# SauersML/genomic_pca

Measured on AMD Instinct MI355X. Metric: SNPs x samples / sec through rSVD at k=20; max|dPC| vs ref, higher is better.
Workload: dtype i8 (exact: int8 dosages x 4 signed 7-bit fixed-point digit planes of the skinny operand, i32 accumulate, f64 recombination; accuracy >= f32)

## Files before the change

### genomic_pca_amd/_lib.py

```python
from __future__ import annotations

import ctypes as C
import os
import subprocess

_PKG = os.path.dirname(os.path.abspath(__file__))
LIB_PATH = os.path.join(_PKG, "libgpca.so")
CSRC = os.path.join(_PKG, "csrc")

GPCA_OK = 0
GPCA_ERR_BAD_ARG = -1
GPCA_ERR_OOM = -2
GPCA_ERR_HIP = -3
GPCA_ERR_RCCL = -4
GPCA_ERR_MISSING_GENOTYPE = -5
GPCA_ERR_NOT_CONVERGED = -6
GPCA_ERR_STATE = -7
GPCA_ERR_NO_DEVICE = -8
GPCA_ERR_INVALID_GENOTYPE = -9
GPCA_UNIQUE_ID_BYTES = 128
PREC_DEFAULT = 0
PREC_I8_EXACT = 1
PREC_F32_MFMA = 2
STORE_AUTO = 0
STORE_2BIT = 1
STORE_INT8 = 2
GRM_STANDARDIZED = 0
GRM_CENTRED = 1
CFG_SIMPLE_KERNELS = 1
CFG_NO_COMPACT = 2
CFG_NO_NARROW = 4
CFG_NO_SPIN_SYNC = 8


class GpcaLibraryError(RuntimeError):
    pass


class GpcaError(RuntimeError):
    def __init__(self, status: int, message: str):
        super().__init__(f"[gpca status {status}] {message}")
        self.status = status
        self.message = message


class gpca_config(C.Structure):
    _fields_ = [("device", C.c_int32), ("precision", C.c_int32), ("storage", C.c_int32), ("digit_planes", C.c_int32),
# ... 137 lines not shown
```

### genomic_pca_amd/csrc/gemm_i8.hip

```cpp
#include "gemm_i8_common.h"

namespace gpca {

template <int NSU>
struct GqnG { i32x4 g[4 * NSU]; float r, b; };
template <int NSU>
__device__ __forceinline__ void gqn_load(GqnG<NSU>& b, const int8_t* __restrict__ G, int64_t ldg, int64_t unit, int c, int h,
                                         const float* __restrict__ rv, const float* __restrict__ bv) {
    const __amdgpu_buffer_rsrc_t rg = make_rsrc8(G + unit * 32 * ldg);
    const uint32_t vo = (uint32_t)(c * ldg + 16 * h);
#pragma unroll
    for (int j = 0; j < 4 * NSU; ++j) b.g[j] = __builtin_amdgcn_raw_buffer_load_b128(rg, vo, 32u * j, 2);
    b.r = rv[unit * 32 + c]; b.b = bv[unit * 32 + c];
}
template <int NSU, int PF>
__global__ __launch_bounds__(256, 1) void k_gq_n(const int8_t* __restrict__ G, int64_t ldg, int64_t units,
                                                  const int8_t* __restrict__ Qd, const double* __restrict__ qscale,
                                                  const float* __restrict__ rv, const float* __restrict__ bv,
                                                  const float* __restrict__ sv, float* __restrict__ Tout,
                                                  float* __restrict__ cunit, double* __restrict__ apart, int scale_out, int64_t ldt) {
    const int lane = threadIdx.x & 63;
    const int wv = __builtin_amdgcn_readfirstlane(threadIdx.x >> 6);
    const int c = lane & 31, h = lane >> 5;
    const int64_t wave = (int64_t)blockIdx.x * 4 + wv, waves = (int64_t)gridDim.x * 4;
// ... 591 lines not shown
    if (h == 0) apart[((int64_t)blockIdx.x * 4 + wv) * 32 + c] = (double)am;
}

int launch_gq_d(hipStream_t st, const int8_t* G, int64_t ldg, const GqPlan& plan, int64_t Npad, const int8_t* Qd,
                const double* qscale, const float* r, const float* b, const float* s, float* Tout, float* cpart, double* apart,
                int scale_out, int64_t ldt, const KernelOpts& ko) {
    if (!dma_shape_ok(Npad, 256, plan.units * 32, 32) || ldg < Npad) return (int)hipErrorInvalidValue;
    const dim3 grid((unsigned)(plan.waves / 4)), blk(256);
    const int64_t nstage = Npad / 128;
    int phase = ko.gq_phase;
    if (phase < 0) phase = (nstage >= 16 && nstage <= 400) ? (int)((nstage / 8) << 16) : 0;
    hipLaunchKernelGGL((k_gq_d<1>), grid, blk, sizeof(GqdSmem), st, G, ldg, plan.units, nstage, Qd, qscale, r, b, s, Tout, cpart, apart, scale_out, ldt, ko.gq_chain, phase);
    return 0;
}

template <bool PACKED>
struct GttXG { unsigned g[16]; };

#ifndef GPCA_GTTX_AUX
#define GPCA_GTTX_AUX 2
#endif
template <bool PACKED>
__device__ __forceinline__ void gttx_load_g(GttXG<PACKED>& b, __amdgpu_buffer_rsrc_t rg, uint32_t gvo, uint32_t row_off, uint32_t ldr) {
#pragma unroll
    for (int i = 0; i < 16; ++i) b.g[i] = (unsigned)__builtin_amdgcn_raw_buffer_load_b32(rg, gvo, row_off + (uint32_t)i * ldr, PACKED ? 0 : GPCA_GTTX_AUX);
}
template <bool PACKED, int ABL = 0>
__device__ __forceinline__ void gttx_decode_step(const GttXG<PACKED>& bn, Gtt2Ops& on, unsigned (&x)[4], unsigned (&y)[4], int m, unsigned bsh) {
    const int w = m >> 2, ph = m & 3;
    if (ABL & 1) { on.bt[ph][w] = (int)bn.g[4 * w + ph]; return; }
// ... 365 lines not shown

int launch_gtt_d(hipStream_t st, const int8_t* G, int64_t ldg, int64_t Mpad, int64_t Npad, const int8_t* Td, double* Ypart,
                 const Gtt8Plan& plan, const KernelOpts& ko) {
    if (plan.tasks_per_wg < 1 || plan.S * 128 != Mpad || !dma_shape_ok(Npad, 256, Mpad, kGQRowsPerWave) || ldg < Npad) return (int)hipErrorInvalidValue;
    const dim3 grid((unsigned)plan.grid), blk(256);
    const int remap = ko.gtt_xcd;
    hipLaunchKernelGGL((k_gtt_d<1>), grid, blk, sizeof(GqdSmem), st, (const uint8_t*)G, ldg, Npad, Td, Ypart, plan.S, plan.C, plan.ngroups, plan.W, plan.tasks_per_wg, plan.strided, remap);
    return 0;
}

int init_device_kernels_i8() {
    int e = 0;
#define GPCA_OPT_IN(KERNEL, BYTES) \
    if (e == 0) e = (int)hipFuncSetAttribute(reinterpret_cast<const void*>(KERNEL), hipFuncAttributeMaxDynamicSharedMemorySize, (int)(BYTES));
    GPCA_OPT_IN((k_gq_d<1>), sizeof(GqdSmem))
    GPCA_OPT_IN((k_gtt_p<kDigits>), sizeof(GtpSmem)) GPCA_OPT_IN((k_gtt_p<3>), sizeof(GtpSmem))
    GPCA_OPT_IN((k_gtt_d<1>), sizeof(GqdSmem))
#undef GPCA_OPT_IN
    return e;
}

}
```

### genomic_pca_amd/csrc/gpca_api.cpp

```cpp
#include "gpca_internal.h"

using namespace gpca;

RcclApi g_rccl;
thread_local std::string g_last_global_err;

static thread_local uint64_t g_tls_err_gen = 0;
static thread_local std::string g_tls_err;
static std::atomic<uint64_t> g_next_gen{1};
int fail(gpca_handle* h, int code, const std::string& msg) {
    if (h) { h->err = msg; g_tls_err_gen = h->gen; g_tls_err = msg; } else g_last_global_err = msg;
    return code;
}

void fold_timings(gpca_handle* h) {
    for (auto& r : h->recs) {
        float ms = 0.f;
        if (hipEventSynchronize(r.b) == hipSuccess && hipEventElapsedTime(&ms, r.a, r.b) == hipSuccess) {
            size_t i = 0;
            for (; i < h->agg.size(); ++i) if (r.name == h->agg[i].name) break;
            if (i == h->agg.size()) { gpca_kernel_timing t{}; snprintf(t.name, sizeof t.name, "%s", r.name.c_str()); h->agg.push_back(t); }
            h->agg[i].launches++; h->agg[i].total_ms += ms; h->agg[i].flops += r.flops; h->agg[i].bytes += r.bytes;
        }
        h->ev_pool.push_back(r.a); h->ev_pool.push_back(r.b);
// ... 41 lines not shown
    h->storage_cfg = cfg ? cfg->storage : GPCA_STORE_AUTO;
    if (h->storage_cfg != GPCA_STORE_AUTO && h->storage_cfg != GPCA_STORE_INT8 && h->storage_cfg != GPCA_STORE_2BIT) { delete h; return fail(nullptr, GPCA_ERR_BAD_ARG, "gpca_create: unknown storage mode"); }
    if (h->precision != GPCA_PREC_F32_MFMA && h->precision != GPCA_PREC_I8_EXACT) { delete h; return fail(nullptr, GPCA_ERR_BAD_ARG, "gpca_create: unknown precision mode"); }
    h->storage = h->storage_cfg == GPCA_STORE_2BIT ? GPCA_STORE_2BIT : GPCA_STORE_INT8;
    {
        const int dp = cfg ? cfg->digit_planes : 0;
        if (dp != 0 && dp != 3 && dp != 4) { delete h; return fail(nullptr, GPCA_ERR_BAD_ARG, "gpca_create: digit_planes must be 0, 3 or 4"); }
        if (dp == 3 && !(h->precision == GPCA_PREC_I8_EXACT && h->storage_cfg == GPCA_STORE_2BIT)) { delete h; return fail(nullptr, GPCA_ERR_BAD_ARG, "gpca_create: digit_planes = 3 is implemented for GPCA_PREC_I8_EXACT with GPCA_STORE_2BIT"); }
        h->nd_cfg = dp;
        h->nd = dp == 3 ? 3 : ((dp == 0 && h->precision == GPCA_PREC_I8_EXACT && h->storage == GPCA_STORE_2BIT) ? 3 : 4);
    }
    {
        const int32_t flags = cfg ? cfg->reserved[0] : 0, gqw = cfg ? cfg->reserved[1] : 0, gtw = cfg ? cfg->reserved[2] : 0;
        if ((flags & ~GPCA_CFG_ALL) != 0 || gqw < 0 || gtw < 0 || (cfg && cfg->reserved[3] != 0)) { delete h; return fail(nullptr, GPCA_ERR_BAD_ARG, "gpca_create: unknown bits in gpca_config.reserved"); }
        h->simple_kernels = (flags & GPCA_CFG_SIMPLE_KERNELS) != 0;
        h->compact_ok = (flags & GPCA_CFG_NO_COMPACT) == 0;
        h->narrow_ok = (flags & GPCA_CFG_NO_NARROW) == 0;
        h->spin_sync = (flags & GPCA_CFG_NO_SPIN_SYNC) == 0;
        if (gqw) h->gq_waves_target = std::max(4, (int)gqw);
        if (gtw) h->gtt_waves_target = std::max(4, (int)gtw);
    }
    if (hipSetDevice(dev) != hipSuccess || hipStreamCreateWithFlags(&h->st, hipStreamNonBlocking) != hipSuccess) {
        delete h; return fail(nullptr, GPCA_ERR_HIP, "gpca_create: hipSetDevice/hipStreamCreate failed");
    }
    hipDeviceProp_t prop;
    if (hipGetDeviceProperties(&prop, dev) == hipSuccess) {
        if (strncmp(prop.gcnArchName, "gfx950", 6) != 0) {
            std::string m = std::string("gpca_create: device is ") + prop.gcnArchName + ", this library only carries gfx950 code";
            (void)hipStreamDestroy(h->st); delete h; return fail(nullptr, GPCA_ERR_NO_DEVICE, m);
        }
// ... 468 lines not shown
```

### genomic_pca_amd/csrc/gpca_internal.h

```cpp
#pragma once
#include "../../include/gpca.h"
#include "kernels.h"

#include <dlfcn.h>
#include <hip/hip_runtime.h>

#include <algorithm>
#include <atomic>
#include <chrono>
#include <condition_variable>
#include <deque>
#include <thread>
#include <cmath>
#include <cstdio>
#include <cstdlib>
#include <cstring>
#include <map>
#include <mutex>
#include <string>
#include <vector>

using namespace gpca;

typedef struct ncclComm* ncclComm_t;
// ... 142 lines not shown
        hipStream_t st = nullptr;
        hipEvent_t dep = nullptr;
        int64_t *d_rows = nullptr, *d_cols = nullptr; float* d_out = nullptr; unsigned long long* d_err = nullptr;
        size_t cap_rows = 0, cap_cols = 0, cap_out = 0;
    };
    std::mutex pull_mu;
    std::condition_variable pull_cv;
    std::vector<PullLane*> lanes_free;
    int lanes_total = 0;
    std::atomic<int> pulls_in_flight{0};
    double *dYpart64 = nullptr, *d_qscale = nullptr, *d_qinv = nullptr, *d_tscale = nullptr, *d_tinv = nullptr;
    size_t cap_Qd = 0, cap_Td = 0, cap_Ypart64 = 0;
    int nd = 4;
    uint64_t gen = 0;
    int simple_kernels = 0;
    int narrow_ok = 1;
    int gq_waves_target = 1024, gtt_waves_target = 2048;

    gpca_handle* child = nullptr;
    bool child_valid = false, rsvd_on_child = false;
    bool is_child = false;
    const int64_t* d_row_ids = nullptr;
    int compact_ok = 1;

    int world = 1, rank = 0;
    int64_t snp_offset = 0;
    ncclComm_t comm = nullptr;
    gpca_allreduce_fn hook = nullptr;
    void* hook_user = nullptr;
    std::vector<double> hook_buf;
// ... 168 lines not shown
```

### genomic_pca_amd/csrc/gpca_rsvd.cpp

```cpp
#include "gpca_internal.h"

using namespace gpca;

static void tred2(int n, double* V, double* d, double* e) {
    for (int j = 0; j < n; ++j) d[j] = V[(n - 1) * n + j];
    for (int i = n - 1; i > 0; --i) {
        double scale = 0.0, h = 0.0;
        for (int k = 0; k < i; ++k) scale += std::fabs(d[k]);
        if (scale == 0.0) {
            e[i] = d[i - 1];
            for (int j = 0; j < i; ++j) { d[j] = V[(i - 1) * n + j]; V[i * n + j] = 0.0; V[j * n + i] = 0.0; }
        } else {
            for (int k = 0; k < i; ++k) { d[k] /= scale; h += d[k] * d[k]; }
            double f = d[i - 1];
            double g = std::sqrt(h);
            if (f > 0) g = -g;
            e[i] = scale * g; h -= f * g; d[i - 1] = f - g;
            for (int j = 0; j < i; ++j) e[j] = 0.0;
            for (int j = 0; j < i; ++j) {
                f = d[j]; V[j * n + i] = f; g = e[j] + V[j * n + j] * f;
                for (int k = j + 1; k <= i - 1; ++k) { g += V[k * n + j] * d[k]; e[k] += V[k * n + j] * f; }
                e[j] = g;
            }
            f = 0.0;
// ... 122 lines not shown
    return GPCA_OK;
}


static inline bool narrow_shape(const gpca_handle* h) {
    return h->narrow_ok && h->precision == GPCA_PREC_I8_EXACT && h->storage == GPCA_STORE_INT8 && h->N <= kNarrowSamples;
}
static inline bool k2_batched(const gpca_handle* h) {
    return !narrow_shape(h) && !h->simple_kernels;
}
static inline Gtt8Plan k2_plan(const gpca_handle* h, int64_t rows_pad) {
    return narrow_shape(h) ? gtt8_plan_narrow(rows_pad, h->N, std::min(h->gtt_waves_target, 1024)) :
           k2_batched(h) ? gtt8_plan_batched(rows_pad, h->ldg, h->gtt_waves_target) : gtt8_plan(rows_pad, h->ldg, h->gtt_waves_target);
}

static inline GqPlan k1_plan(const gpca_handle* h, int64_t rows_pad) { return gq_plan(rows_pad, h->gq_waves_target); }

static int k2_panel(gpca_handle* h, const PanelView& pv, const int8_t* Td_half, const Gtt8Plan& plan) {
    const int8_t* Td = Td_half + (size_t)(pv.row0 >> 5) * kPlaneBytesPerBlock;
    const bool packed = h->storage == GPCA_STORE_2BIT;
    if (narrow_shape(h)) launch_gtt_n(h->st, pv.g8, h->ld8, pv.rows_pad, h->ldg, Td, h->dYpart64, plan);
    else if (h->simple_kernels) {
        if (packed) launch_gtt_2bit(h->st, pv.g2, h->ld2, pv.rows_pad, h->ldg, Td, h->dYpart64, plan, h->nd);
        else launch_gtt_i8(h->st, pv.g8, h->ld8, pv.rows_pad, h->ldg, Td, h->dYpart64, plan, h->ko);
    } else if (packed) {
        const int e = launch_gtt_p(h->st, pv.g2, h->ld2, pv.rows_pad, h->ldg, Td, h->dYpart64, plan, h->nd, h->ko);
        if (e != 0) return fail(h, GPCA_ERR_HIP, "k_gtt_p launch failed (hip error " + std::to_string(e) + ")");
    } else {
        const int e = launch_gtt_d(h->st, pv.g8, h->ld8, pv.rows_pad, h->ldg, Td, h->dYpart64, plan, h->ko);
        if (e != 0) return fail(h, GPCA_ERR_HIP, "k_gtt_d launch failed (hip error " + std::to_string(e) + ")");
// ... 56 lines not shown

static int stage_AQ(gpca_handle* h, int scale_out) {
    const double elems = (double)h->M * (double)h->N;
    if (h->precision == GPCA_PREC_I8_EXACT) {
        const int L = h->L, halves = L / 32;
        const bool packed = h->storage == GPCA_STORE_2BIT, streamed = h->sm.on;
        const size_t qhalf = (size_t)h->ldg * 32 * kDigits;
        const size_t chalf = (size_t)h->Mpad;
        const size_t ahalf = (size_t)h->gqplan.waves * 32;
        if (streamed && scale_out) HIPCHK(hipMemsetAsync(h->d_amax_run, 0, kMaxSketch * 8, h->st));
        {
            const double by = packed ? elems / 4 : elems;
            ScopedTimer sweep(h, "gemm_GQ", 2.0 * elems * h->l, by * halves, nullptr, streamed);
            CHK(for_each_panel(h, [&](const PanelView& pv) -> int {
                const GqPlan plan = streamed ? k1_plan(h, pv.rows_pad) : h->gqplan;
                for (int hf = 0; hf < halves; ++hf) {
                    const int8_t* Qd = h->dQd + hf * qhalf;
                    const double* qsc = h->d_qscale + 32 * hf;
                    const float* s32 = h->d_s32 + 32 * hf;
                    const float* rr = h->d_r + pv.row0; const float* bb = h->d_b + pv.row0;
                    float* Th = h->dT + (size_t)pv.row0 * L + 32 * hf;
                    float* cp = h->d_cpart + hf * chalf + (size_t)pv.row0;
                    double* ap = h->d_apart + hf * ahalf;
                    ScopedTimer t(h, "gemm_GQ", 2.0 * elems * h->l / halves, by, nullptr, !streamed);
                    if (packed) launch_gq_2bit(h->st, pv.g2, h->ld2, plan, h->ldg, Qd, qsc, rr, bb, s32, Th, cp, ap, scale_out, h->nd, L);
                    else if (narrow_shape(h)) {
                        const int e = launch_gq_n(h->st, pv.g8, h->ld8, plan, h->N, Qd, qsc, rr, bb, s32, Th, cp, ap, scale_out, L);
                        if (e != 0) return fail(h, GPCA_ERR_HIP, "k_gq_n launch failed (hip error " + std::to_string(e) + ")");
                    }
                    else if (!h->simple_kernels) {
                        const int e = launch_gq_d(h->st, pv.g8, h->ld8, plan, h->ldg, Qd, qsc, rr, bb, s32, Th, cp, ap, scale_out, L, h->ko);
                        if (e != 0) return fail(h, GPCA_ERR_HIP, "k_gq_d launch failed (hip error " + std::to_string(e) + ")");
                    }
                    else launch_gq_i8(h->st, pv.g8, h->ld8, plan, h->N, Qd, qsc, rr, bb, s32, Th, cp, scale_out, L, h->ko);
                    HIPCHK(hipGetLastError());
                    if (streamed && scale_out && (packed || !h->simple_kernels || narrow_shape(h))) {
                        launch_absmax_fold(h->st, ap, plan.waves, h->d_amax_run + 32 * hf);
                        HIPCHK(hipGetLastError());
                    }
                }
                return GPCA_OK;
            }));
        }
        h->apart_valid = scale_out != 0 && (packed || !h->simple_kernels || narrow_shape(h));
        h->c_fold_pending = scale_out != 0 && !streamed && h->apart_valid;
        if (scale_out)
            for (int hf = 0; hf < halves; ++hf) {
                if (h->c_fold_pending)
                    launch_post_k1(h->st, h->d_cpart + hf * chalf, h->Mpad / 32, h->d_scratch64 + (size_t)hf * kPostK1Scratch, h->d_apart + hf * ahalf, h->gqplan.waves,
                                   h->d_tscale + 32 * hf, h->d_tinv + 32 * hf, h->nd);
                else launch_sum_partials_f32(h->st, h->d_cpart + hf * chalf, h->Mpad / 32, 32, h->d_c + 32 * hf, h->d_scratch64);
                HIPCHK(hipGetLastError());
            }
        for (int hf = 0; hf < kMaxSketch / 32; ++hf) h->apart_src[hf] = streamed ? h->d_amax_run + 32 * hf : h->d_apart + hf * ahalf;
// ... 12 lines not shown
}

static int stage_power_fused(gpca_handle* h) {
    const double elems = (double)h->M * (double)h->N;
    const int L = h->L, halves = L / 32;
    const bool packed = h->storage == GPCA_STORE_2BIT;
    const size_t qhalf = (size_t)h->ldg * 32 * kDigits, chalf = (size_t)h->Mpad, ahalf = (size_t)h->gqplan.waves * 32;
    const size_t td_half = (size_t)h->Mpad * 32 * kDigits, yint_half = (size_t)h->N * 32;
    {
        const double by = packed ? elems / 4 : elems;
        ScopedTimer sweep(h, "gemm_fused", 4.0 * elems * h->l, by * halves);
        CHK(for_each_panel(h, [&](const PanelView& pv) -> int {
            const GqPlan plan1 = k1_plan(h, pv.rows_pad);
            const Gtt8Plan plan2 = k2_plan(h, pv.rows_pad);
            const float* rr = h->d_r + pv.row0; const float* bb = h->d_b + pv.row0;
            for (int hf = 0; hf < halves; ++hf) {
                const int8_t* Qd = h->dQd + hf * qhalf;
                float* Th = h->dT + (size_t)pv.row0 * L + 32 * hf;
                float* cp = h->d_cpart + hf * chalf + (size_t)pv.row0;
                double* ap = h->d_apart + hf * ahalf;
                if (packed) launch_gq_2bit(h->st, pv.g2, h->ld2, plan1, h->ldg, Qd, h->d_qscale + 32 * hf, rr, bb, h->d_s32 + 32 * hf, Th, cp, ap, 1, h->nd, L);
                else if (narrow_shape(h)) {
                    const int e = launch_gq_n(h->st, pv.g8, h->ld8, plan1, h->N, Qd, h->d_qscale + 32 * hf, rr, bb, h->d_s32 + 32 * hf, Th, cp, ap, 1, L);
                    if (e != 0) return fail(h, GPCA_ERR_HIP, "k_gq_n launch failed (hip error " + std::to_string(e) + ")");
                }
                else {
                    const int e = launch_gq_d(h->st, pv.g8, h->ld8, plan1, h->ldg, Qd, h->d_qscale + 32 * hf, rr, bb, h->d_s32 + 32 * hf, Th, cp, ap, 1, L, h->ko);
                    if (e != 0) return fail(h, GPCA_ERR_HIP, "k_gq_d launch failed (hip error " + std::to_string(e) + ")");
                }
                HIPCHK(hipGetLastError());
                launch_quantize_f32_premax(h->st, Th, pv.rows_pad, pv.rows_pad, ap, plan1.waves, h->d_tscale + 32 * hf, h->d_tinv + 32 * hf,
                                           h->dTd + hf * td_half + (size_t)(pv.row0 >> 5) * kPlaneBytesPerBlock, 0, h->nd, L);
                HIPCHK(hipGetLastError());
            }
            for (int hf = 0; hf < halves; ++hf) {
                CHK(k2_panel(h, pv, h->dTd + hf * td_half, plan2));
                launch_accum_y_scaled(h->st, h->dYpart64, plan2.W, h->ldg, h->N, h->d_tscale + 32 * hf, h->d_yint + hf * yint_half, pv.index == 0);
                HIPCHK(hipGetLastError());
            }
            return GPCA_OK;
        }));
    }
    for (int hf = 0; hf < halves; ++hf) {
        launch_sum_partials_f32(h->st, h->d_cpart + hf * chalf, h->Mpad / 32, 32, h->d_c + 32 * hf, h->d_scratch64);
        HIPCHK(hipGetLastError());
        launch_finish_y_sum(h->st, h->d_yint + hf * yint_half, h->N, h->d_c + 32 * hf, h->dY + 32 * hf, L);
        HIPCHK(hipGetLastError());
    }
// ... 220 lines not shown
    return 2 * npad <= h->Mpad;
}
static int ensure_child(gpca_handle* h) {
    if (h->child && h->child_valid) return GPCA_OK;
    drop_child(h);
    const bool packed = h->storage == GPCA_STORE_2BIT;
    const int64_t n = h->n_pca, npad = round_up(n, kGQRowsPerWave), pitch = packed ? h->ld2 : h->ld8;
    size_t free_b = 0, total_b = 0;
    HIPCHK(hipMemGetInfo(&free_b, &total_b));
    const double need = (double)npad * (double)pitch + (double)npad * 1024.0 + (double)h->ldg * 8192.0 + 1073741824.0;
    if (need > (double)free_b) return GPCA_ERR_OOM;
    gpca_handle* c = new gpca_handle();
    c->is_child = true; c->compact_ok = 0;
    c->device = h->device; c->precision = h->precision; c->storage = h->storage; c->nd = h->nd; c->ko = h->ko;
    c->st = h->st;
    c->simple_kernels = h->simple_kernels; c->narrow_ok = h->narrow_ok; c->spin_sync = h->spin_sync;
    c->gq_waves_target = h->gq_waves_target; c->gtt_waves_target = h->gtt_waves_target;
    c->timing_on = h->timing_on;
    c->M = n; c->N = h->N; c->Mpad = npad; c->ldg = h->ldg; c->ld8 = h->ld8; c->ld2 = h->ld2; c->cap_rows_pad = npad; c->pack_flags = h->pack_flags;
    h->child = c;
    auto build = [&]() -> int {
        gpca_handle* hh = h;
        (void)hh;
        if (packed) { HIPCHK(malloc_genotypes(h, (void**)&c->dG2, (size_t)npad * (size_t)pitch)); }
        else { HIPCHK(malloc_genotypes(h, (void**)&c->dG, (size_t)npad * (size_t)pitch)); }
        char* gdst = packed ? (char*)c->dG2 : (char*)c->dG;
        if (npad > n) HIPCHK(hipMemsetAsync(gdst + (size_t)n * pitch, 0, (size_t)(npad - n) * pitch, h->st));
        launch_gather_rows(h->st, packed ? (const void*)h->dG2 : (const void*)h->dG, pitch, h->d_pca_rows, n, gdst);
        HIPCHK(hipGetLastError());
        {
            gpca_handle* h = c;
// ... 378 lines not shown
```

### genomic_pca_amd/csrc/kernels.h

```cpp
#pragma once
#include <hip/hip_runtime.h>
#include <stdint.h>
#include "eig_result.h"
#include "plan_math.h"

namespace gpca {

struct QcParams { double min_call_rate, min_maf, max_hwe_p; };

struct KernelOpts {
    int gq_phase = -1;
    int gq_chain = 1;
    int gtt_xcd = 1;
};
int init_device_kernels_i8();
int init_device_kernels_common();
int init_device_kernels_eig();

void launch_small_eigh(hipStream_t st, const double* src, int nslices, int n, int L, int k, int zmode, double denom, const int* cholflag,
                       double* Z, double* res, double* Vout);

__host__ __device__ inline int64_t blocked_t_index(int64_t row, int col, int LT) {
    const int64_t group = row >> 4;
    const int w = (int)(row & 15), lt = col >> 5, cc = col & 31;
// ... 137 lines not shown
void launch_quantize_f64_prescaled(hipStream_t st, const double* X, int64_t rows, int64_t rows_pad, const double* inv, int8_t* Xd, int layout, int nd = 4, int64_t ldx = 32);
void launch_quantize_f64_finishq(hipStream_t st, const double* X, int64_t rows, int64_t rows_pad, int8_t* Xd, int layout, int nd, int64_t ldx,
                                 const double* csum_part, const double* amax_part, int64_t P, int ldp, double* s64, float* s32, double* scale, double* inv);
void launch_quantize_f32_premax(hipStream_t st, const float* X, int64_t rows, int64_t rows_pad, const double* apart, int64_t P,
                                double* scale, double* inv, int8_t* Xd, int layout, int nd = 4, int64_t ldx = 32);
void launch_post_k1(hipStream_t st, const float* cpart, int64_t units, double* cscratch, const double* apart, int64_t P, double* scale, double* inv, int nd);
void launch_quantize_f32_cfold(hipStream_t st, const float* X, int64_t rows, int64_t rows_pad, const double* inv, int8_t* Xd, int layout, int nd,
                               int64_t ldx, const double* cscratch, int cslices, double* c);
int launch_gtt_p(hipStream_t st, const uint8_t* G2, int64_t ld2, int64_t Mpad, int64_t Npad, const int8_t* Td, double* Ypart,
                 const Gtt8Plan& plan, int nd = 4, const KernelOpts& ko = KernelOpts());
int launch_gtt_d(hipStream_t st, const int8_t* G, int64_t ldg, int64_t Mpad, int64_t Npad, const int8_t* Td, double* Ypart,
                 const Gtt8Plan& plan, const KernelOpts& ko = KernelOpts());
int launch_gq_d(hipStream_t st, const int8_t* G, int64_t ldg, const GqPlan& plan, int64_t Npad, const int8_t* Qd,
                const double* qscale, const float* r, const float* b, const float* s, float* Tout, float* cpart, double* apart,
                int scale_out, int64_t ldt = 32, const KernelOpts& ko = KernelOpts());
void launch_gtt_2bit(hipStream_t st, const uint8_t* G2, int64_t ld2, int64_t Mpad, int64_t Npad, const int8_t* Td,
                     double* Ypart, const Gtt8Plan& plan, int nd = 4);


void launch_project(hipStream_t st, const void* G, int packed, int64_t ldr, int64_t Mpad, int64_t Npad, const int8_t* Ta, const int8_t* Tb,
                    const uint32_t* rmask, double* Ypa, double* Ypb, unsigned* cnt, unsigned* bad, const PrjPlan& plan, int nd, int lazy_b);
void launch_project_correct(hipStream_t st, const double* Yint_b, int64_t N, const double* tscale_b, const unsigned* cnt, int64_t n_model,
                            double* Y, int64_t ldy);
void launch_project_colmax(hipStream_t st, const float* X, int64_t rows, int L, unsigned long long* out);
void launch_project_used(hipStream_t st, const unsigned* cnt, int64_t N, double n_model, double* used);

constexpr int kGrmDigits = 6;
constexpr int kGrmFlushRows = 4096;
constexpr int kGrmTabBytes = 4 * kGrmDigits * 32;
void launch_grm(hipStream_t st, const void* G, int packed, int64_t ldr, int64_t rows_pad, const int8_t* tab, const uint32_t* kmask,
// ... 52 lines not shown
```

### include/gpca.h

```cpp
#ifndef GPCA_H
#define GPCA_H

#include <stddef.h>
#include <stdint.h>

#if defined(__GNUC__)
#define GPCA_API __attribute__((visibility("default")))
#else
#define GPCA_API
#endif

#ifdef __cplusplus
extern "C" {
#endif

#define GPCA_VERSION 250
#define GPCA_MISSING_I8 (-127)

typedef struct gpca_handle gpca_handle;

typedef enum gpca_status {
    GPCA_OK = 0,
    GPCA_ERR_BAD_ARG = -1,
    GPCA_ERR_OOM = -2,
// ... 17 lines not shown
    GPCA_STORE_2BIT = 1,
    GPCA_STORE_INT8 = 2
} gpca_storage;

typedef struct gpca_config {
    int32_t device;
    int32_t precision;
    int32_t storage;
    int32_t digit_planes;
    int32_t reserved[4];
} gpca_config;
#define GPCA_CFG_SIMPLE_KERNELS 1
#define GPCA_CFG_NO_COMPACT 2
#define GPCA_CFG_NO_NARROW 4
#define GPCA_CFG_NO_SPIN_SYNC 8
#define GPCA_CFG_ALL 15

typedef struct gpca_qc_config {
    double min_snp_call_rate;
    double min_snp_maf;
    double max_snp_hwe_p_value;
} gpca_qc_config;

GPCA_API int gpca_version(void);
GPCA_API const char* gpca_status_string(int status);
GPCA_API int gpca_create(const gpca_config* cfg, gpca_handle** out);
GPCA_API int gpca_destroy(gpca_handle* h);
GPCA_API const char* gpca_last_error(gpca_handle* h);

GPCA_API int gpca_upload_genotypes_i8(gpca_handle* h, const int8_t* snp_major, int64_t M, int64_t N, int64_t ld);
GPCA_API int gpca_upload_bed2bit(gpca_handle* h, const uint8_t* bed_rows, int64_t M, int64_t N);
// ... 141 lines not shown
```

Before: 964.7 billion.

## Fuse both Q column halves into one int8 GEMM pass over genotypes

Adds a k_gq_d2 kernel that computes the G·Q product for two 32-column halves of the skinny operand in a single sweep over the int8 genotype matrix. Before, each half launched its own kernel that re-read G. The intent is to halve genotype memory traffic on the memory-bound first GEMM of each rSVD iteration. The new kernel has its own LDS layout, a slot-based DMA pipeline with compile-time audited vmcnt waits, and chaining across rounds. It runs by default for int8 non-narrow storage, with a config flag to fall back to per-half launches. The cost is a larger LDS footprint, more accumulator registers per wave, and a complex hand-tuned wait schedule.

Result: no change. 964.7 billion (median of 2 runs) (+0.0%).

```diff
diff --git a/genomic_pca_amd/_lib.py b/genomic_pca_amd/_lib.py
--- a/genomic_pca_amd/_lib.py
+++ b/genomic_pca_amd/_lib.py
@@ -31,6 +31,7 @@
 CFG_NO_COMPACT = 2
 CFG_NO_NARROW = 4
 CFG_NO_SPIN_SYNC = 8
+CFG_K1_PER_HALF = 16
 
 
 class GpcaLibraryError(RuntimeError):
diff --git a/genomic_pca_amd/csrc/gemm_i8.hip b/genomic_pca_amd/csrc/gemm_i8.hip
--- a/genomic_pca_amd/csrc/gemm_i8.hip
+++ b/genomic_pca_amd/csrc/gemm_i8.hip
@@ -1,4 +1,5 @@
 #include "gemm_i8_common.h"
+#include "gqd2_counts.h"
 
 namespace gpca {
 
@@ -629,6 +630,247 @@
     return 0;
 }
 
+struct Gqd2Smem {
+    i32x4 q[2][kGqd2Blocks][4][kDigits][64];
+    i32x4 g[4][kGqd2Slots][256];
+    float tile[4][32 * 32];
+    float rb[4][2][32 * kGqd2MaxR];
+    double colq[4][kGqd2Blocks][32];
+    float cols[4][kGqd2Blocks][32];
+};
+static_assert(sizeof(Gqd2Smem) <= 160 * 1024, "LDS of one CU");
+static_assert(kGqd2MaxR * kGqd2Blocks * kDigits * 16 == 256, "accumulators of a wave");
+static_assert(32 * kGqd2MaxR <= 64, "r and b of a round's rows: one 64-dword DMA each");
+
+__device__ __forceinline__ void gqd2_wait_young(int batches) {
+    switch (batches) {
+        case 1: gqd_wait_vm<gqd2_young_wait(1)>(); break;
+        case 2: gqd_wait_vm<gqd2_young_wait(2)>(); break;
+        default: gqd_wait_vm<gqd2_young_wait(3)>(); break;
+    }
+}
+static_assert(gqd2_q_young(1, 0) <= 3 && gqd2_q_young(2, 0) <= 3 && gqd2_q_young(2, 1) >= 1 && gqd2_q_young_early(1) >= 1, "cases of gqd2_wait_young");
+
+template <int NT, int R>
+__device__ __forceinline__ void gqd2_round(const int8_t* __restrict__ G, int64_t ldg, int64_t nstage,
+                                           const int8_t* __restrict__ Qd0, const int8_t* __restrict__ Qd1, Gqd2Smem* sm, int wv, int lane, int c, int h,
+                                           int64_t unit0, int nvalid, bool prologue, bool chain, GqdRound nx, uint32_t& rslot, uint32_t ph,
+                                           int64_t rows_total, const float* __restrict__ rv,
+                                           const float* __restrict__ bv, float* __restrict__ Tout, int scale_out, int64_t ldt,
+                                           float* __restrict__ cunit, int64_t c_stride, float (&amax)[kGqd2Blocks]) {
+    constexpr int S = kGqd2Slots, B = kGqd2Blocks;
+    static_assert(R >= 1 && R <= kGqd2MaxR, "tiles per wave");
+    auto phys = [&](uint32_t st_) -> uint32_t { const uint32_t p_ = st_ + ph; return p_ >= (uint32_t)nstage ? p_ - (uint32_t)nstage : p_; };
+    const int64_t row0 = unit0 * 32;
+    const i32x4 rg = gqd_rsrc(G + row0 * ldg);
+    const i32x4 rgn = gqd_rsrc(G + nx.unit0 * 32 * ldg);
+    const i32x4 rq0 = gqd_rsrc(Qd0 + wv * 1024), rq1 = gqd_rsrc(Qd1 + wv * 1024);
+    const uint32_t ld32 = (uint32_t)ldg;
+    const uint32_t gvo_e = (uint32_t)(lane >> 3) * ld32 + 16u * (uint32_t)((lane & 7) ^ (lane >> 4));
+    const uint32_t gvo_o = (uint32_t)(lane >> 3) * ld32 + 16u * (uint32_t)((lane & 7) ^ (lane >> 4) ^ 4);
+    const uint32_t qvo = (uint32_t)(lane * 16);
+    uint32_t toff[R];
+#pragma unroll
+    for (int t = 0; t < R; ++t) toff[t] = (uint32_t)(t < nvalid ? 32 * t : 0) * ld32;
+    {
+        const uint32_t lds_rb = (uint32_t)(uintptr_t)(__attribute__((address_space(3))) void*)&sm->rb[wv][0][0];
+        i32x4 rr_ = gqd_rsrc(rv + row0), rb_ = gqd_rsrc(bv + row0);
+        rr_.z = rb_.z = (int)((rows_total - row0) * 4);
+        asm volatile("s_waitcnt lgkmcnt(0)" ::: "memory");
+        gqd_dma_dword(lds_rb, qvo >> 2, rr_, 0u);
+        gqd_dma_dword(lds_rb + 4u * 32u * kGqd2MaxR, qvo >> 2, rb_, 0u);
+    }
+    constexpr uint32_t QCH = kDigits * 1024;
+    const uint32_t lds_q = (uint32_t)(uintptr_t)(__attribute__((address_space(3))) void*)&sm->q[0][0][0][0][0] + (uint32_t)wv * 1024u;
+    const uint32_t lds_g = (uint32_t)(uintptr_t)(__attribute__((address_space(3))) void*)&sm->g[0][0][0] + (uint32_t)wv * (S * 4096u);
+    const char* gl = reinterpret_cast<const char*>(&sm->g[wv][0][0]);
+    uint32_t loff[4];
+#pragma unroll
+    for (int s4 = 0; s4 < 4; ++s4) loff[s4] = (uint32_t)(c * 128 + (((2 * s4 + h) ^ ((c >> 1) & 7)) * 16));
+
+    i32x16 acc[R][B][kDigits];
+#pragma unroll
+    for (int t = 0; t < R; ++t)
+#pragma unroll
+        for (int b = 0; b < B; ++b)
+#pragma unroll
+            for (int d = 0; d < kDigits; ++d)
+#pragma unroll
+                for (int e = 0; e < 16; ++e) acc[t][b][d][e] = 0;
+
+#define GQD2_ISSUE_G(RSRC, SO, SLOT)                                                                      \
+    {                                                                                                     \
+        const uint32_t so_ = (SO);                                                                        \
+        const uint32_t la_ = lds_g + (uint32_t)(SLOT) * 4096u;                                            \
+        _Pragma("unroll") for (int i = 0; i < kGqd2FillDmas; ++i) gqd_dma<NT>(la_ + 1024u * i, (i & 1) ? gvo_o : gvo_e, RSRC, so_ + 8u * i * ld32); \
+    }
+#define GQD2_ISSUE_Q(ST, QS)                                                                              \
+    {                                                                                                     \
+        const uint32_t sq_ = phys((uint32_t)(ST)) * 4u;                                                   \
+        _Pragma("unroll") for (int j = 0; j < 4; ++j)                                                     \
+            gqd_dma(lds_q + (uint32_t)((((QS) * B + 0) * 4 + j) * kDigits) * 1024u, qvo, rq0, (sq_ + j) * QCH); \
+        _Pragma("unroll") for (int j = 0; j < 4; ++j)                                                     \
+            gqd_dma(lds_q + (uint32_t)((((QS) * B + 1) * 4 + j) * kDigits) * 1024u, qvo, rq1, (sq_ + j) * QCH); \
+    }
+    int64_t ist = 0;
+    int it = 0;
+    bool in_next = false;
+    uint32_t pst = 0; int pt = 0;
+#define GQD2_ISSUE_NEXT(SLOT)                                                                             \
+    {                                                                                                     \
+        if (!in_next) {                                                                                   \
+            GQD2_ISSUE_G(rg, toff[it] + phys((uint32_t)ist) * 128u, SLOT)                                 \
+            if (++it == R) { it = 0; if (++ist == nstage) { if (chain) in_next = true; else ist = 0; } }  \
+        } else {                                                                                          \
+            const uint32_t tn_ = (uint32_t)(pt < nx.nv ? 32 * pt : 0) * ld32;                             \
+            GQD2_ISSUE_G(rgn, tn_ + phys(pst) * 128u, SLOT)                                               \
+            if (++pt == nx.R) { pt = 0; ++pst; }                                                          \
+        }                                                                                                 \
+    }
+    if (prologue) {
+        rslot = 0;
+#pragma unroll
+        for (int sl = 0; sl < S - 2; ++sl) GQD2_ISSUE_NEXT(sl)
+        GQD2_ISSUE_Q(0, 0)
+#pragma unroll
+        for (int sl = S - 2; sl < S; ++sl) GQD2_ISSUE_NEXT(sl)
+    } else {
+        ist = S / R; it = S % R;
+    }
+    i32x4 gcur, gnxt;
+
+    for (int64_t st = 0; st < nstage; ++st) {
+        asm volatile("s_waitcnt vmcnt(%0)\n\ts_barrier" :: "n"(gqd2_stage_wait(R)) : "memory");
+        GQD2_ISSUE_Q(st + 1 < nstage ? st + 1 : 0, (int)((st + 1) & 1))
+        i32x4 q[B][4][kDigits];
+#pragma unroll
+        for (int b = 0; b < B; ++b)
+#pragma unroll
+            for (int s4 = 0; s4 < 4; ++s4)
+#pragma unroll
+                for (int d = 0; d < kDigits; ++d) q[b][s4][d] = sm->q[st & 1][b][s4][d][lane];
+        if (st == 0) {
+            gcur = *reinterpret_cast<const i32x4*>(gl + rslot * 4096u + loff[0]);
+            gnxt = *reinterpret_cast<const i32x4*>(gl + rslot * 4096u + loff[1]);
+        }
+#pragma unroll
+        for (int t = 0; t < R; ++t) {
+            const char* ub = gl + rslot * 4096u;
+            const uint32_t nslot = rslot == S - 1 ? 0u : rslot + 1u;
+#pragma unroll
+            for (int s4 = 0; s4 < 4; ++s4) {
+                i32x4 gfar;
+                if (s4 < 2) {
+                    gfar = *reinterpret_cast<const i32x4*>(ub + loff[s4 + 2]);
+                } else {
+                    if (s4 == 2) {
+                        if (st < gqd2_early_stages(R)) gqd2_wait_young(gqd2_q_young_early(R));
+                        else gqd2_wait_young(gqd2_q_young(R, t));
+                    }
+                    gfar = *reinterpret_cast<const i32x4*>(gl + nslot * 4096u + loff[s4 - 2]);
+                }
+#pragma unroll
+                for (int b = 0; b < B; ++b)
+#pragma unroll
+                    for (int d = 0; d < kDigits; ++d)
+                        acc[t][b][d] = __builtin_amdgcn_mfma_i32_32x32x32_i8(gcur, q[b][s4][d], acc[t][b][d], 0, 0, 0);
+                if (s4 == 3) {
+                    asm volatile("" :: "v"(gcur));
+                    GQD2_ISSUE_NEXT(rslot)
+                }
+                gcur = gnxt; gnxt = gfar;
+            }
+            rslot = nslot;
+        }
+    }
+    if (!chain) asm volatile("s_waitcnt vmcnt(0)\n\ts_barrier" ::: "memory");
+#undef GQD2_ISSUE_NEXT
+#undef GQD2_ISSUE_G
+#undef GQD2_ISSUE_Q
+    float* tile = sm->tile[wv];
+#pragma unroll
+    for (int t = 0; t < R; ++t)
+        if (t < nvalid) {
+#pragma unroll
+            for (int b = 0; b < B; ++b)
+                gq_tile_out<7, true>(acc[t][b], 0.f, 0.f, &sm->rb[wv][0][32 * t], &sm->rb[wv][1][32 * t], sm->colq[wv][b][c], sm->cols[wv][b][c], scale_out, tile, Tout + 32 * b, ldt, unit0 + t,
+                                     cunit + b * c_stride, amax[b], lane, nx.unit0 != unit0);
+        }
+}
+
+template <int NT>
+__global__ __launch_bounds__(256, 1) void k_gq_d2(const int8_t* __restrict__ G, int64_t ldg, int64_t units, int64_t nstage,
+                                                   const int8_t* __restrict__ Qd, int64_t qd_stride, const double* __restrict__ qscale,
+                                                   const float* __restrict__ rv, const float* __restrict__ bv,
+                                                   const float* __restrict__ sv, float* __restrict__ Tout,
+                                                   float* __restrict__ cpart, int64_t c_stride, double* __restrict__ apart, int64_t a_stride,
+                                                   int scale_out, int64_t ldt, int chain_ok, int phase_mul) {
+    extern __shared__ __attribute__((aligned(16))) char gqd_smem[];
+    Gqd2Smem* sm = reinterpret_cast<Gqd2Smem*>(gqd_smem);
+    __builtin_assume(nstage >= 2 && (nstage & 1) == 0);
+    const int wv = __builtin_amdgcn_readfirstlane(threadIdx.x >> 6);
+    const uint32_t ph = (uint32_t)(((int64_t)(blockIdx.x & 7) * (phase_mul & 0xffff) + (int64_t)(blockIdx.x >> 3) * (phase_mul >> 16)) % nstage);
+    const int64_t u0 = (units * (int64_t)blockIdx.x) / gridDim.x;
+    const int64_t u1 = (units * ((int64_t)blockIdx.x + 1)) / gridDim.x;
+    float amax[kGqd2Blocks] = {0.f, 0.f};
+    {
+        const int l0 = threadIdx.x & 63;
+        sm->colq[wv][l0 >> 5][l0 & 31] = qscale[l0];
+        sm->cols[wv][l0 >> 5][l0 & 31] = sv[l0];
+    }
+    auto round_at = [&](int64_t u) -> GqdRound {
+        const int64_t rem = u1 - u, take = rem < kGqd2RoundUnits ? rem : kGqd2RoundUnits;
+        const int base = (int)(take >> 2), extra = (int)(take & 3);
+        const int nv = base + (wv < extra ? 1 : 0);
+        GqdRound r;
+        r.nv = nv; r.R = nv ? nv : 1;
+        r.unit0 = nv ? u + wv * base + (wv < extra ? wv : extra) : u;
+        return r;
+    };
+    const bool chain_all = chain_ok && nstage > kGqd2Slots;
+    uint32_t rslot = 0;
+    int64_t u = u0;
+    while (u < u1) {
+        const int64_t un = u + (u1 - u < kGqd2RoundUnits ? u1 - u : kGqd2RoundUnits);
+        const GqdRound cur = round_at(u);
+        const bool chain = chain_all && un < u1;
+        const bool prologue = !chain_all || u == u0;
+        GqdRound nx = cur;
+        if (chain) nx = round_at(un);
+        int lane;
+        asm volatile("v_mbcnt_lo_u32_b32 %0, -1, 0\n\tv_mbcnt_hi_u32_b32 %0, -1, %0" : "=v"(lane));
+        const int c = lane & 31, h = lane >> 5;
+#define GPCA_GQD2_ROUND(RR) gqd2_round<NT, RR>(G, ldg, nstage, Qd, Qd + qd_stride, sm, wv, lane, c, h, cur.unit0, cur.nv, prologue, chain, nx, rslot, ph, units * 32, rv, bv, Tout, scale_out, ldt, cpart, c_stride, amax)
+        if (cur.R == 2) GPCA_GQD2_ROUND(2);
+        else GPCA_GQD2_ROUND(1);
+#undef GPCA_GQD2_ROUND
+        u = un;
+    }
+#pragma unroll
+    for (int b = 0; b < kGqd2Blocks; ++b) {
+        float am_lo, am_hi; halves_pair(amax[b], am_lo, am_hi);
+        const float am = fmaxf(am_lo, am_hi);
+        int l0;
+        asm volatile("v_mbcnt_lo_u32_b32 %0, -1, 0\n\tv_mbcnt_hi_u32_b32 %0, -1, %0" : "=v"(l0));
+        if (l0 < 32) apart[b * a_stride + ((int64_t)blockIdx.x * 4 + wv) * 32 + l0] = (double)am;
+    }
+}
+
+int launch_gq_d2(hipStream_t st, const int8_t* G, int64_t ldg, const GqPlan& plan, int64_t Npad, const int8_t* Qd, int64_t qd_stride,
+                 const double* qscale, const float* r, const float* b, const float* s, float* Tout, float* cpart, int64_t c_stride,
+                 double* apart, int64_t a_stride, int scale_out, int64_t ldt, const KernelOpts& ko) {
+    if (!dma_shape_ok(Npad, 256, plan.units * 32, 32) || ldg < Npad) return (int)hipErrorInvalidValue;
+    if (ldt < 32 * kGqd2Blocks || qd_stride < Npad * 32 * kDigits || qd_stride % 1024 != 0) return (int)hipErrorInvalidValue;
+    if (c_stride < plan.units * 32 || a_stride < plan.waves * 32 || plan.waves < 4 || plan.waves % 4 != 0) return (int)hipErrorInvalidValue;
+    const dim3 grid((unsigned)(plan.waves / 4)), blk(256);
+    const int64_t nstage = Npad / 128;
+    int phase = ko.gq_phase;
+    if (phase < 0) phase = (nstage >= 16 && nstage <= 400) ? (int)((nstage / 8) << 16) : 0;
+    hipLaunchKernelGGL((k_gq_d2<1>), grid, blk, sizeof(Gqd2Smem), st, G, ldg, plan.units, nstage, Qd, qd_stride, qscale, r, b, s, Tout, cpart, c_stride, apart, a_stride,
+                       scale_out, ldt, ko.gq_chain, phase);
+    return 0;
+}
+
 template <bool PACKED>
 struct GttXG { unsigned g[16]; };
 
@@ -1024,6 +1266,7 @@
 #define GPCA_OPT_IN(KERNEL, BYTES) \
     if (e == 0) e = (int)hipFuncSetAttribute(reinterpret_cast<const void*>(KERNEL), hipFuncAttributeMaxDynamicSharedMemorySize, (int)(BYTES));
     GPCA_OPT_IN((k_gq_d<1>), sizeof(GqdSmem))
+    GPCA_OPT_IN((k_gq_d2<1>), sizeof(Gqd2Smem))
     GPCA_OPT_IN((k_gtt_p<kDigits>), sizeof(GtpSmem)) GPCA_OPT_IN((k_gtt_p<3>), sizeof(GtpSmem))
     GPCA_OPT_IN((k_gtt_d<1>), sizeof(GqdSmem))
 #undef GPCA_OPT_IN
diff --git a/genomic_pca_amd/csrc/gpca_api.cpp b/genomic_pca_amd/csrc/gpca_api.cpp
--- a/genomic_pca_amd/csrc/gpca_api.cpp
+++ b/genomic_pca_amd/csrc/gpca_api.cpp
@@ -79,6 +79,7 @@
         const int32_t flags = cfg ? cfg->reserved[0] : 0, gqw = cfg ? cfg->reserved[1] : 0, gtw = cfg ? cfg->reserved[2] : 0;
         if ((flags & ~GPCA_CFG_ALL) != 0 || gqw < 0 || gtw < 0 || (cfg && cfg->reserved[3] != 0)) { delete h; return fail(nullptr, GPCA_ERR_BAD_ARG, "gpca_create: unknown bits in gpca_config.reserved"); }
         h->simple_kernels = (flags & GPCA_CFG_SIMPLE_KERNELS) != 0;
+        h->k1_per_half = (flags & GPCA_CFG_K1_PER_HALF) != 0;
         h->compact_ok = (flags & GPCA_CFG_NO_COMPACT) == 0;
         h->narrow_ok = (flags & GPCA_CFG_NO_NARROW) == 0;
         h->spin_sync = (flags & GPCA_CFG_NO_SPIN_SYNC) == 0;
diff --git a/genomic_pca_amd/csrc/gpca_internal.h b/genomic_pca_amd/csrc/gpca_internal.h
--- a/genomic_pca_amd/csrc/gpca_internal.h
+++ b/genomic_pca_amd/csrc/gpca_internal.h
@@ -180,6 +180,7 @@
     int nd = 4;
     uint64_t gen = 0;
     int simple_kernels = 0;
+    int k1_per_half = 0;
     int narrow_ok = 1;
     int gq_waves_target = 1024, gtt_waves_target = 2048;
 
diff --git a/genomic_pca_amd/csrc/gpca_rsvd.cpp b/genomic_pca_amd/csrc/gpca_rsvd.cpp
--- a/genomic_pca_amd/csrc/gpca_rsvd.cpp
+++ b/genomic_pca_amd/csrc/gpca_rsvd.cpp
@@ -160,6 +160,9 @@
            k2_batched(h) ? gtt8_plan_batched(rows_pad, h->ldg, h->gtt_waves_target) : gtt8_plan(rows_pad, h->ldg, h->gtt_waves_target);
 }
 
+static inline bool k1_one_read(const gpca_handle* h) {
+    return h->storage != GPCA_STORE_2BIT && !narrow_shape(h) && !h->simple_kernels && !h->k1_per_half;
+}
 static inline GqPlan k1_plan(const gpca_handle* h, int64_t rows_pad) { return gq_plan(rows_pad, h->gq_waves_target); }
 
 static int k2_panel(gpca_handle* h, const PanelView& pv, const int8_t* Td_half, const Gtt8Plan& plan) {
@@ -246,7 +249,8 @@
             ScopedTimer sweep(h, "gemm_GQ", 2.0 * elems * h->l, by * halves, nullptr, streamed);
             CHK(for_each_panel(h, [&](const PanelView& pv) -> int {
                 const GqPlan plan = streamed ? k1_plan(h, pv.rows_pad) : h->gqplan;
-                for (int hf = 0; hf < halves; ++hf) {
+                for (int hf = 0, nb = 1; hf < halves; hf += nb) {
+                    nb = (k1_one_read(h) && hf + 1 < halves) ? 2 : 1;
                     const int8_t* Qd = h->dQd + hf * qhalf;
                     const double* qsc = h->d_qscale + 32 * hf;
                     const float* s32 = h->d_s32 + 32 * hf;
@@ -254,8 +258,12 @@
                     float* Th = h->dT + (size_t)pv.row0 * L + 32 * hf;
                     float* cp = h->d_cpart + hf * chalf + (size_t)pv.row0;
                     double* ap = h->d_apart + hf * ahalf;
-                    ScopedTimer t(h, "gemm_GQ", 2.0 * elems * h->l / halves, by, nullptr, !streamed);
-                    if (packed) launch_gq_2bit(h->st, pv.g2, h->ld2, plan, h->ldg, Qd, qsc, rr, bb, s32, Th, cp, ap, scale_out, h->nd, L);
+                    ScopedTimer t(h, "gemm_GQ", 2.0 * elems * h->l / halves * nb, by, nullptr, !streamed);
+                    if (nb == 2) {
+                        const int e = launch_gq_d2(h->st, pv.g8, h->ld8, plan, h->ldg, Qd, (int64_t)qhalf, qsc, rr, bb, s32, Th, cp, (int64_t)chalf, ap, (int64_t)ahalf, scale_out, L, h->ko);
+                        if (e != 0) return fail(h, GPCA_ERR_HIP, "k_gq_d2 launch failed (hip error " + std::to_string(e) + ")");
+                    }
+                    else if (packed) launch_gq_2bit(h->st, pv.g2, h->ld2, plan, h->ldg, Qd, qsc, rr, bb, s32, Th, cp, ap, scale_out, h->nd, L);
                     else if (narrow_shape(h)) {
                         const int e = launch_gq_n(h->st, pv.g8, h->ld8, plan, h->N, Qd, qsc, rr, bb, s32, Th, cp, ap, scale_out, L);
                         if (e != 0) return fail(h, GPCA_ERR_HIP, "k_gq_n launch failed (hip error " + std::to_string(e) + ")");
@@ -266,10 +274,11 @@
                     }
                     else launch_gq_i8(h->st, pv.g8, h->ld8, plan, h->N, Qd, qsc, rr, bb, s32, Th, cp, scale_out, L, h->ko);
                     HIPCHK(hipGetLastError());
-                    if (streamed && scale_out && (packed || !h->simple_kernels || narrow_shape(h))) {
-                        launch_absmax_fold(h->st, ap, plan.waves, h->d_amax_run + 32 * hf);
-                        HIPCHK(hipGetLastError());
-                    }
+                    if (streamed && scale_out && (packed || !h->simple_kernels || narrow_shape(h)))
+                        for (int b = 0; b < nb; ++b) {
+                            launch_absmax_fold(h->st, ap + b * ahalf, plan.waves, h->d_amax_run + 32 * (hf + b));
+                            HIPCHK(hipGetLastError());
+                        }
                 }
                 return GPCA_OK;
             }));
@@ -312,12 +321,17 @@
             const GqPlan plan1 = k1_plan(h, pv.rows_pad);
             const Gtt8Plan plan2 = k2_plan(h, pv.rows_pad);
             const float* rr = h->d_r + pv.row0; const float* bb = h->d_b + pv.row0;
-            for (int hf = 0; hf < halves; ++hf) {
+            for (int hf = 0, nb = 1; hf < halves; hf += nb) {
+                nb = (k1_one_read(h) && hf + 1 < halves) ? 2 : 1;
                 const int8_t* Qd = h->dQd + hf * qhalf;
                 float* Th = h->dT + (size_t)pv.row0 * L + 32 * hf;
                 float* cp = h->d_cpart + hf * chalf + (size_t)pv.row0;
                 double* ap = h->d_apart + hf * ahalf;
-                if (packed) launch_gq_2bit(h->st, pv.g2, h->ld2, plan1, h->ldg, Qd, h->d_qscale + 32 * hf, rr, bb, h->d_s32 + 32 * hf, Th, cp, ap, 1, h->nd, L);
+                if (nb == 2) {
+                    const int e = launch_gq_d2(h->st, pv.g8, h->ld8, plan1, h->ldg, Qd, (int64_t)qhalf, h->d_qscale + 32 * hf, rr, bb, h->d_s32 + 32 * hf, Th, cp, (int64_t)chalf, ap, (int64_t)ahalf, 1, L, h->ko);
+                    if (e != 0) return fail(h, GPCA_ERR_HIP, "k_gq_d2 launch failed (hip error " + std::to_string(e) + ")");
+                }
+                else if (packed) launch_gq_2bit(h->st, pv.g2, h->ld2, plan1, h->ldg, Qd, h->d_qscale + 32 * hf, rr, bb, h->d_s32 + 32 * hf, Th, cp, ap, 1, h->nd, L);
                 else if (narrow_shape(h)) {
                     const int e = launch_gq_n(h->st, pv.g8, h->ld8, plan1, h->N, Qd, h->d_qscale + 32 * hf, rr, bb, h->d_s32 + 32 * hf, Th, cp, ap, 1, L);
                     if (e != 0) return fail(h, GPCA_ERR_HIP, "k_gq_n launch failed (hip error " + std::to_string(e) + ")");
@@ -327,9 +341,11 @@
                     if (e != 0) return fail(h, GPCA_ERR_HIP, "k_gq_d launch failed (hip error " + std::to_string(e) + ")");
                 }
                 HIPCHK(hipGetLastError());
-                launch_quantize_f32_premax(h->st, Th, pv.rows_pad, pv.rows_pad, ap, plan1.waves, h->d_tscale + 32 * hf, h->d_tinv + 32 * hf,
-                                           h->dTd + hf * td_half + (size_t)(pv.row0 >> 5) * kPlaneBytesPerBlock, 0, h->nd, L);
-                HIPCHK(hipGetLastError());
+                for (int b = 0; b < nb; ++b) {
+                    launch_quantize_f32_premax(h->st, Th + 32 * b, pv.rows_pad, pv.rows_pad, ap + b * ahalf, plan1.waves, h->d_tscale + 32 * (hf + b), h->d_tinv + 32 * (hf + b),
+                                               h->dTd + (hf + b) * td_half + (size_t)(pv.row0 >> 5) * kPlaneBytesPerBlock, 0, h->nd, L);
+                    HIPCHK(hipGetLastError());
+                }
             }
             for (int hf = 0; hf < halves; ++hf) {
                 CHK(k2_panel(h, pv, h->dTd + hf * td_half, plan2));
@@ -580,7 +596,7 @@
     c->is_child = true; c->compact_ok = 0;
     c->device = h->device; c->precision = h->precision; c->storage = h->storage; c->nd = h->nd; c->ko = h->ko;
     c->st = h->st;
-    c->simple_kernels = h->simple_kernels; c->narrow_ok = h->narrow_ok; c->spin_sync = h->spin_sync;
+    c->simple_kernels = h->simple_kernels; c->k1_per_half = h->k1_per_half; c->narrow_ok = h->narrow_ok; c->spin_sync = h->spin_sync;
     c->gq_waves_target = h->gq_waves_target; c->gtt_waves_target = h->gtt_waves_target;
     c->timing_on = h->timing_on;
     c->M = n; c->N = h->N; c->Mpad = npad; c->ldg = h->ldg; c->ld8 = h->ld8; c->ld2 = h->ld2; c->cap_rows_pad = npad; c->pack_flags = h->pack_flags;
diff --git a/genomic_pca_amd/csrc/gqd2_counts.h b/genomic_pca_amd/csrc/gqd2_counts.h
--- /dev/null
+++ b/genomic_pca_amd/csrc/gqd2_counts.h
@@ -0,0 +1,63 @@
+#ifndef GPCA_GQD2_COUNTS_H
+#define GPCA_GQD2_COUNTS_H
+
+namespace gpca {
+
+constexpr int kGqd2Slots = 4;
+constexpr int kGqd2Blocks = 2;
+constexpr int kGqd2MaxR = 2;
+constexpr int kGqd2FillDmas = 4;
+constexpr int kGqd2PlaneDmas = 4 * kGqd2Blocks;
+constexpr int kGqd2RoundUnits = 4 * kGqd2MaxR;
+
+constexpr int gqd2_stage_wait(int R) { return kGqd2FillDmas * R; }
+constexpr int gqd2_q_young(int R, int t) {
+    int n = 0;
+    for (int j = 0; j <= kGqd2Slots - 2; ++j) n += (((t - j) % R + R) % R == 0) ? 1 : 0;
+    return n;
+}
+constexpr int gqd2_early_stages(int R) { return R == 1 ? 2 : 0; }
+constexpr int gqd2_q_young_early(int R) { return R == 1 ? 2 : gqd2_q_young(R, 1); }
+constexpr int gqd2_young_wait(int batches) { return kGqd2FillDmas * (kGqd2Slots - 2) + kGqd2PlaneDmas * batches; }
+constexpr int gqd2_unit_wait(int R, int st, int t) {
+    return gqd2_young_wait(st < gqd2_early_stages(R) ? gqd2_q_young_early(R) : gqd2_q_young(R, t));
+}
+constexpr int kGqd2VmcntMax = 63;
+
+constexpr int gqd2_audit(int nfull, int Rlast, int nstage, int tight_from) {
+    constexpr int S = kGqd2Slots, kMaxUnits = 1024, kMaxStages = 512;
+    if ((nfull + 1) * nstage * kGqd2MaxR + S >= kMaxUnits || (nfull + 1) * nstage + 1 >= kMaxStages) return -1;
+    int fill_end[kMaxUnits] = {};
+    int q_end[kMaxStages] = {};
+    int issued = 0, nf = 0;
+    for (int i = 0; i < S - 2; ++i) { issued += kGqd2FillDmas; fill_end[nf++] = issued; }
+    issued += kGqd2PlaneDmas; q_end[0] = issued;
+    for (int i = S - 2; i < S; ++i) { issued += kGqd2FillDmas; fill_end[nf++] = issued; }
+    int m = 0, gs = 0;
+    for (int rnd = 0; rnd <= nfull; ++rnd) {
+        const int R = rnd < nfull ? kGqd2MaxR : Rlast;
+        for (int st = 0; st < nstage; ++st, ++gs) {
+            if (gqd2_stage_wait(R) > issued - q_end[gs]) return 1000 + rnd;
+            if (st >= tight_from && gqd2_stage_wait(R) != issued - q_end[gs]) return 2000 + rnd;
+            issued += kGqd2PlaneDmas; q_end[gs + 1] = issued;
+            for (int t = 0; t < R; ++t, ++m) {
+                const int w = gqd2_unit_wait(R, st, t), young = issued - fill_end[m + 1];
+                if (w > kGqd2VmcntMax) return 3000 + rnd;
+                if (w > young) return 4000 + rnd;
+                if (st >= tight_from && w != young) return 5000 + rnd;
+                issued += kGqd2FillDmas; fill_end[nf++] = issued;
+            }
+        }
+    }
+    return 0;
+}
+static_assert(gqd2_audit(0, 2, 2, 2) == 0 && gqd2_audit(0, 1, 2, 2) == 0 && gqd2_audit(0, 2, 4, 2) == 0 && gqd2_audit(0, 1, 4, 2) == 0, "cold rounds (drained form, 2 and 4 stages)");
+static_assert(gqd2_audit(0, 2, 6, 2) == 0 && gqd2_audit(0, 1, 6, 2) == 0 && gqd2_audit(0, 2, 80, 2) == 0 && gqd2_audit(0, 1, 80, 2) == 0, "cold rounds");
+static_assert(gqd2_audit(1, 2, 6, 2) == 0 && gqd2_audit(1, 1, 6, 2) == 0 && gqd2_audit(3, 2, 8, 2) == 0 && gqd2_audit(3, 1, 8, 2) == 0 && gqd2_audit(2, 1, 80, 2) == 0, "chained rounds");
+static_assert(gqd2_audit(2, 2, 8, 0) == 0, "R = 2: no early stages");
+static_assert(gqd2_stage_wait(2) == 8 && gqd2_stage_wait(1) == 4, "stage start: vmcnt 8 / 4");
+static_assert(gqd2_q_young(2, 0) == 2 && gqd2_q_young(2, 1) == 1 && gqd2_q_young(1, 0) == 3, "batches younger than the next unit");
+static_assert(gqd2_young_wait(1) == 16 && gqd2_young_wait(2) == 24 && gqd2_young_wait(3) == 32, "R = 2: vmcnt 24 / 16; R = 1: 32, its first two stages 24");
+
+}
+#endif
diff --git a/genomic_pca_amd/csrc/kernels.h b/genomic_pca_amd/csrc/kernels.h
--- a/genomic_pca_amd/csrc/kernels.h
+++ b/genomic_pca_amd/csrc/kernels.h
@@ -175,6 +175,9 @@
 int launch_gq_d(hipStream_t st, const int8_t* G, int64_t ldg, const GqPlan& plan, int64_t Npad, const int8_t* Qd,
                 const double* qscale, const float* r, const float* b, const float* s, float* Tout, float* cpart, double* apart,
                 int scale_out, int64_t ldt = 32, const KernelOpts& ko = KernelOpts());
+int launch_gq_d2(hipStream_t st, const int8_t* G, int64_t ldg, const GqPlan& plan, int64_t Npad, const int8_t* Qd, int64_t qd_stride,
+                 const double* qscale, const float* r, const float* b, const float* s, float* Tout, float* cpart, int64_t c_stride,
+                 double* apart, int64_t a_stride, int scale_out, int64_t ldt, const KernelOpts& ko = KernelOpts());
 void launch_gtt_2bit(hipStream_t st, const uint8_t* G2, int64_t ld2, int64_t Mpad, int64_t Npad, const int8_t* Td,
                      double* Ypart, const Gtt8Plan& plan, int nd = 4);
 
diff --git a/include/gpca.h b/include/gpca.h
--- a/include/gpca.h
+++ b/include/gpca.h
@@ -55,7 +55,8 @@
 #define GPCA_CFG_NO_COMPACT 2
 #define GPCA_CFG_NO_NARROW 4
 #define GPCA_CFG_NO_SPIN_SYNC 8
-#define GPCA_CFG_ALL 15
+#define GPCA_CFG_K1_PER_HALF 16
+#define GPCA_CFG_ALL 31
 
 typedef struct gpca_qc_config {
     double min_snp_call_rate;
```
